# VealFang/PLI-SLAM

Hardware: AMD Instinct MI355X
Metric: stereo frames/sec (ORB+LSD extract+match), 752x480 EuRoC (higher is better)
Workload: dtype u8; 1 GPU; 1xMI355X: 752x480 stereo pairs, extract + stereo Hamming match (BASELINE configs[1] shape, batched); 752x480, 1200 ORB kp (8 levels x1.2) + LSD/LBD (<=100 lines); 256 stereo frames per GPU per step; frames_per_gpu=256, parallelism=frame-batch data parallel, 1 rank(s), gather of result tables to rank 0

## Files before the change

pli_slam_amd/csrc/common.hpp:

```cpp
#pragma once
#include <hip/hip_runtime.h>
#include <cstdint>
#include <cstdio>
#include <cstring>
#include <string>
#include <vector>
#include <map>
#include "../../include/pli_frontend.h"

namespace pli {

constexpr int MAX_LEVELS = 16;
constexpr int CELL_CAP = 512;
constexpr int GRID_COLS = 64;
constexpr int GRID_ROWS = 48;
constexpr int LSD_CHUNK = 4096;

struct LevelGeom {
  int w, h, pitch;
  int64_t offset;
  int minBX, minBY, maxBX, maxBY;
  int nCols, nRows, wCell, hCell;
  int cellBase;
  int nfeatures;
// ... 13 lines not shown
  LevelGeom lv[MAX_LEVELS];
  int cellsPerImage, kpSlotsPerImage, candPerImage;
  int64_t pyrBlock;
  int kpCap, klCap;
  int umax[16];
  int LW, LH, lpitch;
  int LWt;
  int g2Thresh;
  int nBins;
  int minRegSize;
  double prec, lsdScale;
  float alignLo, alignHi;
  double hotBand2;
  double rectApproxBand;
  int alignFilter, alignPad;
  int parityFlags, parityPad;
  double rho;
  int maxLines;
  int lsdNFeatures;
  double minLength;
  float bf, maxD;
  int sWs, bestLR;
  double lineSimTh, overlapTh, ratio12L, minDispRatio, minDisp, horizTh;
};

struct alignas(128) RxCtl {
  int state;
  int changed;
  int overflow;
  int rounds;
  int nSmall, nBig;
  int changedOdd;
  int pad0[25];
  int nHand;
  int pad1[31];
  int nextBig;
  int pad2[31];
  unsigned long long rectArena;
  int pad3[30];
  int races;
  int pad4[31];
};
constexpr int RX_ARENA_BITS = 40;

struct RxSeed {
  int rank, xy;
// ... 96 lines not shown
```

pli_slam_amd/csrc/lsd_rect.hpp:

```cpp
#pragma once
#include "kernels.hpp"
#include "device_prims.hpp"

namespace pli {

constexpr double RX_PI = 3.14159265358979323846;
constexpr double RX_DEG2RAD = RX_PI / 180;
constexpr double RX_3_2_PI = (3 * RX_PI) / 2;
constexpr double RX_2PI = 2 * RX_PI;

__device__ __forceinline__ double rx_angle_diff(double a, double b) {
  double diff = a - b;
  while (diff <= -RX_PI) diff += RX_2PI;
  while (diff > RX_PI) diff -= RX_2PI;
  return fabs(diff);
}

constexpr int RX_RECT_GROUP_MAX = 192;
constexpr int RX_RECT_CACHE = 4;

__device__ __forceinline__ void rx_wave_sync() {
  __builtin_amdgcn_fence(__ATOMIC_RELEASE, "wavefront");
  __builtin_amdgcn_wave_barrier();
  __builtin_amdgcn_fence(__ATOMIC_ACQUIRE, "wavefront");
}

template <int LANES>
__device__ __forceinline__ void rx_rect_region(bool on, const RxRect& it, const DevParams& P, const float4* __restrict__ rec,
                                               const double* __restrict__ mg, const int* __restrict__ arena,
                                               float4* __restrict__ rgSeg, double (*st)[64], double (*wc)[64], int (*ec)[64], int rmask,
                                               const int2* __restrict__ hot = nullptr ,
                                               const float2* __restrict__ cold = nullptr ) {
  const int lane = threadIdx.x & 63, gl = lane & (LANES - 1), g0 = lane & ~(LANES - 1);
  const int W = P.LW;
  const double prec = P.prec;
  const int cnt = on ? it.cnt : 0;
  const int* lst = arena + it.off;
  const double reg_angle = (double)fast_atan2_deg(it.sumdy, it.sumdx) * RX_DEG2RAD;
  int cmax = cnt;
#pragma unroll
  for (int o = 32; o >= LANES; o >>= 1) cmax = max(cmax, __shfl_xor(cmax, o, 64));
  double acc = 0.0;
  for (int c0 = 0; c0 < cmax; c0 += LANES) {
    const int kk = c0 + gl;
    double v0 = 0.0, v1 = 0.0, v2 = 0.0;
    if (kk < cnt) {
      const int e = lst[kk];
      const int ex = e & 0xFFFF, ey = e >> 16;
      const double w = mg ? mg[ey * W + ex] : sqrt((double)__float_as_int(rec[ey * W + ex].w) / 4.0);
      v0 = (double)ex * w;
      v1 = (double)ey * w;
      v2 = w;
      if (c0 < RX_RECT_CACHE * LANES) { wc[c0 / LANES][lane] = w; ec[c0 / LANES][lane] = e; }
    }
    rx_wave_sync();
    st[0][lane] = v0; st[1][lane] = v1; st[2][lane] = v2;
    rx_wave_sync();
    if (gl < 3 && c0 < cnt) {
      const int mm = (min(LANES, cnt - c0) + 7) & ~7;
      for (int tt = 0; tt < mm; tt += 8) {
        double a[8];
#pragma unroll
        for (int u = 0; u < 8; ++u) a[u] = st[gl][g0 + tt + u];
#pragma unroll
        for (int u = 0; u < 8; ++u) acc += a[u];
      }
    }
  }
  const double cq = acc / __shfl(acc, g0 + 2, 64);
  const double x = __shfl(cq, g0, 64), y = __shfl(cq, g0 + 1, 64);
  acc = 0.0;
  for (int c0 = 0; c0 < cmax; c0 += LANES) {
    const int kk = c0 + gl;
    double v0 = 0.0, v1 = 0.0, v2 = 0.0;
    if (kk < cnt) {
      const bool cached = c0 < RX_RECT_CACHE * LANES;
      const int e = cached ? ec[c0 / LANES][lane] : lst[kk];
      const int ex = e & 0xFFFF, ey = e >> 16;
      const double w = cached ? wc[c0 / LANES][lane] : (mg ? mg[ey * W + ex] : sqrt((double)__float_as_int(rec[ey * W + ex].w) / 4.0));
      const double dx = (double)ex - x, dy = (double)ey - y;
      v0 = dy * dy * w;
      v1 = dx * dx * w;
      v2 = dx * dy * w;
    }
    rx_wave_sync();
    st[0][lane] = v0; st[1][lane] = v1; st[2][lane] = v2;
    rx_wave_sync();
    if (gl < 3 && c0 < cnt) {
      const int mm = (min(LANES, cnt - c0) + 7) & ~7;
      for (int tt = 0; tt < mm; tt += 8) {
        double a[8];
#pragma unroll
        for (int u = 0; u < 8; ++u) a[u] = st[gl][g0 + tt + u];
        if (gl < 2) {
#pragma unroll
          for (int u = 0; u < 8; ++u) acc += a[u];
        } else {
#pragma unroll
          for (int u = 0; u < 8; ++u) acc -= a[u];
        }
      }
    }
  }
  const double Ixx = __shfl(acc, g0, 64), Iyy = __shfl(acc, g0 + 1, 64), Ixy = __shfl(acc, g0 + 2, 64);
  const double lambda = 0.5 * (Ixx + Iyy - sqrt((Ixx - Iyy) * (Ixx - Iyy) + 4.0 * Ixy * Ixy));
  const bool wide = fabs(Ixx) > fabs(Iyy);
  double theta = (double)fast_atan2_deg(wide ? (float)(lambda - Ixx) : (float)Ixy, wide ? (float)Ixy : (float)(lambda - Iyy));
  theta *= RX_DEG2RAD;
  double adiff = rx_angle_diff(theta, reg_angle);
  {
    const bool need = on && it.approx != 0 && hot != nullptr && fabs(adiff - prec) < P.rectApproxBand;
    if (__builtin_amdgcn_ballot_w64(need)) {
      int cm = need ? cnt : 0;
#pragma unroll
      for (int o = 32; o >= LANES; o >>= 1) cm = max(cm, __shfl_xor(cm, o, 64));
      float sx = 0.f, sy = 0.f;
      for (int c0 = 0; c0 < cm; c0 += LANES) {
        const int kk = c0 + gl;
        float cy = 0.f, cz = 0.f;
        if (need && kk < cnt) {
          const int e = lst[kk];
          const int p = (e >> 16) * W + (e & 0xFFFF);
          if (kk == 0) {
            double sn, cs;
            sincos((double)__int_as_float(hot[p].x) * RX_DEG2RAD, &sn, &cs);
// ... 23 lines not shown
  double l_min = 0, l_max = 0;
  for (int kk = gl; kk < cnt; kk += LANES) {
    const int e = kk < RX_RECT_CACHE * LANES ? ec[kk / LANES][lane] : lst[kk];
    const double l = ((double)(e & 0xFFFF) - x) * dxr + ((double)(e >> 16) - y) * dyr;
    l_max = fmax(l_max, l);
    l_min = fmin(l_min, l);
  }
#pragma unroll
  for (int o = LANES / 2; o > 0; o >>= 1) {
    l_max = fmax(l_max, __shfl_xor(l_max, o, 64));
    l_min = fmin(l_min, __shfl_xor(l_min, o, 64));
  }
  double e = ((gl & 1) ? y : x) + ((gl & 2) ? l_max : l_min) * ((gl & 1) ? dyr : dxr);
  e += 0.5;
  const double scale = P.lsdScale;
  if (scale != 1) e /= scale;
  if (on && gl < 4) reinterpret_cast<float*>(&rgSeg[it.rank & rmask])[gl] = (float)e;
}


__device__ __forceinline__ void rx_rect_wave(const DevParams& P, const RxCtl& c, const float4* __restrict__ rec, const double* __restrict__ mg,
                                             const int* __restrict__ arena, const RxRect* __restrict__ rects, int rectCap,
                                             float4* __restrict__ rgSeg, int first, int stride, double (*st)[64], double (*wc)[64],
                                             int (*ec)[64], int rmask = -1, const int2* __restrict__ hot = nullptr,
                                             const float2* __restrict__ cold = nullptr) {
  const int nrect = min((int)(c.rectArena >> RX_ARENA_BITS), rectCap);
  const int lane = threadIdx.x & 63, g = lane >> 4;
  for (int w0 = first * 4; w0 < nrect; w0 += stride * 4) {
    RxRect it = {0, 0, 0, 1.f, 0.f, 0};
    const bool have = w0 + g < nrect;
    if (have) it = rects[w0 + g];
    const bool small = have && it.cnt <= RX_RECT_GROUP_MAX;
    if (__builtin_amdgcn_ballot_w64(small)) rx_rect_region<16>(small, it, P, rec, mg, arena, rgSeg, st, wc, ec, rmask, hot, cold);
    unsigned long long big = __builtin_amdgcn_ballot_w64(have && !small) & 0x0001000100010001ull;
    while (big) {
      const int gl0 = __ffsll((long long)big) - 1;
      big &= big - 1ull;
      RxRect bt;
      bt.rank = __shfl(it.rank, gl0, 64); bt.off = __shfl(it.off, gl0, 64); bt.cnt = __shfl(it.cnt, gl0, 64);
      bt.sumdx = __shfl(it.sumdx, gl0, 64); bt.sumdy = __shfl(it.sumdy, gl0, 64); bt.approx = __shfl(it.approx, gl0, 64);
      rx_rect_region<64>(true, bt, P, rec, mg, arena, rgSeg, st, wc, ec, rmask, hot, cold);
    }
  }
}

}
```

pli_slam_amd/csrc/lsd_relax.hip:

```cpp
#include "kernels.hpp"
#include "device_prims.hpp"
#include "lsd_rect.hpp"
#include <climits>
#include <type_traits>

namespace pli {

constexpr float RX_NOTDEF = -1024.f;
constexpr int RX_INF = LSD_ID_INF;

__device__ __forceinline__ int2 rx_load_own(const int2* p) {
  unsigned long long v = __hip_atomic_load(reinterpret_cast<const unsigned long long*>(p), __ATOMIC_RELAXED,
                                           __HIP_MEMORY_SCOPE_AGENT);
  return make_int2((int)(v & 0xFFFFFFFFull), (int)(v >> 32));
}

__device__ __forceinline__ int rx_lds_read(const int* p) {
  typedef __attribute__((address_space(3))) const volatile int lds_cvint;
  return *(lds_cvint*)p;
}


__device__ __forceinline__ int rx_block_append(bool flag, int* counter, int* lds) {
  const int tid = threadIdx.x, lane = tid & 63, wv = tid >> 6, nw = blockDim.x >> 6;
// ... 674 lines not shown

__global__ __launch_bounds__(64) void k_rx_grow_wave(const DevParams* __restrict__ Pp, RxCtl* __restrict__ ctl,
                                                     const float4* __restrict__ recAll, int2* __restrict__ ownAll,
                                                     const RxSeed* __restrict__ bigAll, int bigCap,
                                                     const RxHand* __restrict__ handAll, int handCap,
                                                     int* __restrict__ rgSizeAll, int2* __restrict__ rgBoxAll,
                                                     int* __restrict__ arenaAll, int arenaCap,
                                                     RxRect* __restrict__ rectAll, int rectCap, int img0, int t) {
  rx_grow_groups<64, 1024>(Pp, ctl, recAll, ownAll, bigAll, bigCap, handAll, handCap, rgSizeAll, rgBoxAll, arenaAll, arenaCap,
                           rectAll, rectCap, img0, t);
}

#endif

__global__ __launch_bounds__(64) void k_rx_rect(const DevParams* __restrict__ Pp, RxCtl* __restrict__ ctl,
                                                const float4* __restrict__ recAll, const int* __restrict__ arenaAll,
                                                int arenaCap, const RxRect* __restrict__ rectAll, int rectCap,
                                                float4* __restrict__ rgSegAll, int img0, const double* __restrict__ mgAll, int rmask,
                                                const int2* __restrict__ hotAll ,
                                                const float2* __restrict__ coldAll ) {
  __shared__ double st[3][64];
  __shared__ double wc[RX_RECT_CACHE][64];
  __shared__ int ec[RX_RECT_CACHE][64];
  const DevParams& P = *Pp;
  const int img = blockIdx.y + img0;
  const RxCtl& c = ctl[img];
  if (c.state == 2 || c.overflow) return;
  const int64_t npix = (int64_t)P.LW * P.LH;
  rx_rect_wave(P, c, recAll + img * npix, mgAll ? mgAll + img * npix : nullptr ,
               arenaAll + (int64_t)img * arenaCap, rectAll + (int64_t)img * rectCap, rectCap, rgSegAll + img * npix, blockIdx.x, gridDim.x, st, wc, ec, rmask,
               hotAll ? hotAll + img * npix : nullptr, coldAll ? coldAll + img * npix : nullptr);
}

constexpr int RX_CCHUNK = 2048;

__device__ __forceinline__ bool rx_emits(const int* order, const int2* own, int size, int i, int n, int minReg) {
  if (i >= n) return false;
  return size >= minReg && own[order[i]].x == i;
}

__global__ __launch_bounds__(256) void k_rx_count(const RxCtl* __restrict__ ctl, const int* __restrict__ orderAll,
                                                  const int* __restrict__ nDefined, const int2* __restrict__ ownAll,
                                                  const int* __restrict__ rgSizeAll, int* __restrict__ chunkCntAll,
                                                  int nChunks, int64_t npix, int minReg, int img0) {
  __shared__ int wsum[4];
  const int img = blockIdx.y + img0;
  if (ctl[img].state != 2 || ctl[img].overflow) return;
  const int n = nDefined[img];
  const int tid = threadIdx.x;
  int cntv = 0;
  int sz[RX_CCHUNK / 256];
#pragma unroll
  for (int j = 0; j < RX_CCHUNK / 256; ++j) sz[j] = rgSizeAll[img * npix + min((int)blockIdx.x * RX_CCHUNK + j * 256 + tid, max(n - 1, 0))];
// ... 55 lines not shown
```

pli_slam_amd/csrc/lsd_tile.hip:

```cpp
#include "kernels.hpp"
#include "device_prims.hpp"
#include "lsd_rect.hpp"
#include <climits>
#include <type_traits>

namespace pli {

constexpr float TX_NOTDEF = -1024.f;
constexpr int TX_INF = LSD_ID_INF;
constexpr double TX_PI = 3.14159265358979323846;
constexpr double TX_DEG2RAD = TX_PI / 180;
constexpr double TX_3_2_PI = (3 * TX_PI) / 2;
constexpr double TX_2PI = 2 * TX_PI;
#if !defined(PLI_DEV) && (defined(TX_CLAIM_SCOPE) || defined(TX_GROUP) || defined(TX_OWN_LOAD) || defined(TX_DIAG_PAD) || defined(TX_DIAG_NOWAIT) || defined(TX_DIAG_HOT_NOFOLD))
#error "diagnostic builds of lsd_tile.hip need -DPLI_DEV"
#endif
#ifndef TX_CLAIM_SCOPE
#define TX_CLAIM_SCOPE __HIP_MEMORY_SCOPE_AGENT
#endif
#ifndef TX_GROUP
#define TX_GROUP 8
#endif
static_assert(TX_GROUP == 0 || TX_GROUP == 2 || TX_GROUP == 4 || TX_GROUP == 8, "a group member is an octet of lanes");
constexpr int TX_GQ = 768;
// ... 1965 lines not shown
    __builtin_amdgcn_fence(__ATOMIC_RELEASE, "agent");
    __hip_atomic_fetch_add(&bar[0], 1u, __ATOMIC_RELAXED, __HIP_MEMORY_SCOPE_AGENT);
    int ok = 1;
    unsigned spins = 0;
    while (__hip_atomic_load(&bar[0], __ATOMIC_RELAXED, __HIP_MEMORY_SCOPE_AGENT) < target) {
      __builtin_amdgcn_s_sleep(4);
      if ((++spins & 63u) == 0u &&
          (__hip_atomic_load(&bar[32], __ATOMIC_RELAXED, __HIP_MEMORY_SCOPE_AGENT) != 0u || spins > (1u << 21))) {
        __hip_atomic_store(&bar[32], 1u, __ATOMIC_RELAXED, __HIP_MEMORY_SCOPE_AGENT);
        ok = 0;
        break;
      }
    }
    __builtin_amdgcn_fence(__ATOMIC_ACQUIRE, "agent");
    s_ok = ok;
  }
  __syncthreads();
  asm volatile("s_dcache_inv" ::: "memory");
  return s_ok != 0;
}

__global__ __launch_bounds__(256) void k_tx_tail(TxTailArgs A) {
  __shared__ int qs[4][TX_GQ];
  __shared__ int gbs[4][TX_BMAXBLK + 4];
  __shared__ int parks[4][TX_PARK];
  __shared__ double sts[4][3][64];
  __shared__ double wcs[4][RX_RECT_CACHE][64];
  __shared__ int ecs[4][RX_RECT_CACHE][64];
  __shared__ int s_live, s_n;
  __shared__ int s_list[256];
  if (A.forceAbort) {
    if (threadIdx.x == 0) __hip_atomic_store(&A.bar[32], 1u, __ATOMIC_RELAXED, __HIP_MEMORY_SCOPE_AGENT);
    return;
  }
  const DevParams& P = *A.Pp;
  const int W = P.LW, H = P.LH;
  const int64_t npix = (int64_t)W * H;
  const int tid = threadIdx.x, wv = tid >> 6;
  const int G = gridDim.x;
  const int nbx = (W + 31) / 32, nbyA = (A.TH + 7) / 8, nbyB = (H + 31) / 32, ntile = A.ntx * A.nty, ncell = A.TW * A.TH;
  const int64_t nA = (int64_t)nbx * nbyA * A.nimg, nB = (int64_t)nbx * nbyB * A.nimg, nC = (int64_t)ntile * A.nimg;
  const int nwaves = G * 4, gw = blockIdx.x * 4 + wv;
  auto relaxing = [&](int il) -> bool {
    const RxCtl& c = A.ctl[A.img0 + il];
    return c.state != 2 && c.overflow == 0;
  };
// ... 79 lines not shown
        const int64_t va = base + (int64_t)s_list[i] * G;
        const int il = (int)(va / ntile);
        if (A.hot)
          tx_grow_tile<true, false, TX_GQ, 0, true>(A.Pp, A.ctl, A.rec, A.own, A.list, A.tileCnt, A.ts, A.ntx, A.nty, A.rgSize, A.rgBox, A.rgDirty,
                                                    A.tileAct, A.TW, A.TH, A.arena, A.arenaCap, A.rects, A.rectCap, A.img0 + il,
                                                    (int)(va - (int64_t)il * ntile), t, A.rank, A.rgLost, A.tileTouch, A.DL, qs[wv], gbs[wv],
                                                    parks[wv], nullptr, A.hot, A.cold);
        else
        tx_grow_tile<true>(A.Pp, A.ctl, A.rec, A.own, A.list, A.tileCnt, A.ts, A.ntx, A.nty, A.rgSize, A.rgBox, A.rgDirty, A.tileAct, A.TW,
                           A.TH, A.arena, A.arenaCap, A.rects, A.rectCap, A.img0 + il, (int)(va - (int64_t)il * ntile), t, A.rank, A.rgLost,
                           A.tileTouch, A.DL, qs[wv], gbs[wv], parks[wv]);
      }
      __syncthreads();
    }
    if (!tx_grid_barrier(A.bar, ++epoch * G)) return;
    for (int64_t v = (int64_t)blockIdx.x * 256 + tid; v < nC; v += (int64_t)G * 256) A.DL.cnt[(int64_t)A.img0 * ntile + v] = 0;
    {
      const int per = max(1, nwaves / A.nimg);
      for (int il = gw / per; il < A.nimg; il += max(1, nwaves / per)) {
        const int img = A.img0 + il;
        const RxCtl& c = A.ctl[img];
        if (c.state == 2 || c.overflow) continue;
        rx_rect_wave(P, c, A.rec + img * npix, A.mg ? A.mg + img * npix : nullptr, A.arena + (int64_t)img * A.arenaCap,
                     A.rects + (int64_t)img * A.rectCap, A.rectCap, A.rgSeg + img * npix, gw % per, per, sts[wv], wcs[wv], ecs[wv], A.DL.rmask,
                     A.hot ? A.hot + img * npix : nullptr, A.cold ? A.cold + img * npix : nullptr);
      }
    }
    if (!tx_grid_barrier(A.bar, ++epoch * G)) return;
  }
}

}
```

pli_slam_amd/csrc/pli_capi.hip:

```cpp
#include "kernels.hpp"
#include "scratch_plan.hpp"
#include <cmath>
#include <cfloat>
#include <algorithm>
#include <memory>
#include <limits>
#include <cstdlib>
#include <set>
#include <string>
#include <functional>
#include <mutex>
#include <atomic>
#include <dlfcn.h>

using namespace pli;

#ifdef PLI_DEV
#define DEVENV(name) getenv(name)
#else
static inline const char* pli_no_devenv() { return nullptr; }
#define DEVENV(name) (pli_no_devenv())
#endif

namespace {
// ... 6 lines not shown
    if (e__ != hipSuccess) {                                                                 \
      g_err = std::string(#expr) + ": " + hipGetErrorString(e__);                            \
      return PLI_ERR_HIP;                                                                    \
    }                                                                                        \
  } while (0)

inline int64_t alignUp(int64_t v, int64_t a) { return (v + a - 1) / a * a; }
inline int cvRoundf(float v) { return (int)std::nearbyintf(v); }
inline int cvRoundd(double v) { return (int)std::nearbyint(v); }
inline int cvFloorf(float v) { int i = (int)v; return i - (i > v); }

constexpr int RX_AUTO_IMAGES = 2560;
constexpr int TX_SMALL_TILE_WAVES = 12000;

struct ProfEntry { const char* name; hipEvent_t a, b; };

}

struct pli_ctx {
  mutable std::recursive_mutex mu;
  pli_frontend_config cfg;
  DevParams hp;
  DevParams* dP = nullptr;
  int device = 0;
  hipStream_t stream = nullptr;
  bool ownStream = true;
  hipStream_t aux = nullptr;
  hipEvent_t evFork = nullptr, evJoin = nullptr, evLbdPre = nullptr;
  hipStream_t aux2 = nullptr;
  hipEvent_t evRectFork = nullptr, evRectDone = nullptr;
  std::function<pli_status()> sideChain;
  bool lbdPreOnSide = false;
  bool syncDebug = getenv("PLI_SYNC_DEBUG") != nullptr;
  int NI = 0;
  pli_table_layout lay;
  std::vector<void*> allocs;
  uint8_t *pyr = nullptr, *blur = nullptr;
  int* resizeTab[MAX_LEVELS] = {nullptr};
  uint32_t* cellCand = nullptr; int* cellCount = nullptr;
  uint32_t* candAll = nullptr; unsigned short* nodeOf = nullptr; int* candCount = nullptr;
  uint32_t* kpSel = nullptr; int* kpSelCount = nullptr;
  BlurJob *jobOrb = nullptr, *jobLsd = nullptr, *jobLbd = nullptr;
  int orbTiles = 0, l0Tiles = 0;
  uint8_t *tmp8 = nullptr, *lsdScaled = nullptr;
  int64_t tmp8Stride = 0, lsdStride = 0;
  int tmpPitch = 0;
// ... 347 lines not shown
  L.kp_cap = kc; L.kl_cap = lc;
  L.off_counts = take(8 * 4);
  L.off_kp[0] = take((int64_t)kc * sizeof(pli_keypoint));
  L.off_kp[1] = take((int64_t)kc * sizeof(pli_keypoint));
  L.off_desc[0] = take((int64_t)kc * 32);
  L.off_desc[1] = take((int64_t)kc * 32);
  L.off_uright = take((int64_t)kc * 4);
  L.off_depth = take((int64_t)kc * 4);
  L.off_kl[0] = take((int64_t)lc * sizeof(pli_keyline));
  L.off_kl[1] = take((int64_t)lc * sizeof(pli_keyline));
  L.off_ldesc[0] = take((int64_t)lc * 32);
  L.off_ldesc[1] = take((int64_t)lc * 32);
  L.off_disp = take((int64_t)lc * 8);
  L.off_le = take((int64_t)lc * 24);
  L.record_bytes = alignUp(o, 256);
}

pli_status allocAll(pli_ctx* c) {
  const DevParams& P = c->hp;
  const int NI = c->NI;
  pli_status st;
#define A(ptr, n) if ((st = c->dalloc(&(ptr), (size_t)(n))) != PLI_OK) return st
  A(c->dP, 1);
  HIPCHK(hipMemcpy(c->dP, &c->hp, sizeof(DevParams), hipMemcpyHostToDevice));
  A(c->pyr, (size_t)P.pyrBlock * NI);
  for (int l = 1; l < P.nlevels; ++l) {
    const LevelGeom &S = P.lv[l - 1], &D = P.lv[l];
    std::vector<int> t = buildResizeTab(S.w, S.h, D.w, D.h, 1. / ((double)D.w / S.w), 1. / ((double)D.h / S.h));
    A(c->resizeTab[l], t.size());
    HIPCHK(hipMemcpy(c->resizeTab[l], t.data(), t.size() * 4, hipMemcpyHostToDevice));
  }
  A(c->cellCand, (size_t)NI * P.cellsPerImage * CELL_CAP);
  A(c->cellCount, (size_t)NI * P.cellsPerImage);
  A(c->candAll, (size_t)NI * P.candPerImage);
  A(c->nodeOf, (size_t)NI * P.candPerImage);
  A(c->candCount, (size_t)NI * P.nlevels);
  A(c->kpSel, (size_t)NI * P.kpSlotsPerImage);
  A(c->kpSelCount, (size_t)NI * P.nlevels);
  {
    BlurJob J;
    std::memset(&J, 0, sizeof(J));
    J.nplanes = P.nlevels;
    J.radius = ORB_BLUR_R;
    gaussKernelFixed8(2 * ORB_BLUR_R + 1, 2.0, J.k);
    {
      int ksum = 0, kmax = 0;
// ... 444 lines not shown
    if (items)
      LAUNCH(c, "k_lsd_rect", k_lsd_rect, dim3(16, nimg), dim3(64), 0, c->dP, (const LsdRectItem*)items, (const uint2*)c->regScratch,
             (const double*)c->mg, (const double*)c->rectW, (const int*)c->nSeg, c->seg, c->maxSeg, img0);
#endif
  } else {
    const bool trace = DEVENV("PLI_RX_TRACE") != nullptr;
    const bool fullPasses = DEVENV("PLI_RX_FULL") != nullptr;
    const bool perRound = DEVENV("PLI_RX_PROFROUNDS") != nullptr;
    int curT = 0;
    auto rxn = [&](const char* n) -> const char* {
      if (!perRound) return n;
      static std::set<std::string> pool;
      char b[64];
      std::snprintf(b, sizeof(b), "%s@%02d", n, curT);
      return pool.insert(b).first->c_str();
    };
    const int64_t npix64 = (int64_t)npix;
    int growBlocks = std::max(16, std::min(256, 2048 / nimg));
    if (const char* e = DEVENV("PLI_JR_BLOCKS")) growBlocks = std::max(1, atoi(e));
    int bigBlocks = std::max(64, std::min(1024, 16384 / nimg));
    if (const char* e = DEVENV("PLI_JR_BIGBLOCKS")) bigBlocks = std::max(1, atoi(e));
    int rectBlocks = std::max(64, std::min(2048, 32768 / nimg));
    if (const char* e = DEVENV("PLI_RECT_BLOCKS")) rectBlocks = std::max(1, atoi(e));
    int bigThresh = RX_HAND;
    if (const char* e = DEVENV("PLI_JR_BIG")) bigThresh = atoi(e);
    int maxRounds = 96;
    if (const char* e = DEVENV("PLI_RX_MAXROUNDS")) maxRounds = std::max(1, std::min(1 << 20, atoi(e)));
    const float precDeg = (float)(P.prec * 180.0 / 3.14159265358979323846);
    (void)growBlocks; (void)bigBlocks; (void)bigThresh; (void)precDeg;
    if (c->rgClean) HIPCHK(hipMemsetAsync(c->rgClean + (int64_t)img0 * npix, 0, npix64 * nimg, c->stream));
    const bool lostRule = c->lsdMode != 1 && DEVENV("PLI_TX_BOXRULE") == nullptr;
    {
      const int64_t cells = (int64_t)c->tilesW * c->tilesH;
      const int64_t ntile64 = (int64_t)c->txNtx * c->txNty;
      static_assert(sizeof(RxCtl) % 4 == 0, "RxCtl is cleared as words");
      ZeroRanges Z{};
      int zr = 0;
      constexpr int zmax = (int)(sizeof(Z.p) / sizeof(Z.p[0]));
      bool zfull = false;
      auto add = [&](void* p, int64_t words) {
        if (!p || words <= 0) return;
        if (zr == zmax) { zfull = true; return; }
        Z.p[zr] = (uint32_t*)p; Z.words[zr] = words; ++zr;
      };
      add(c->jrCtl + img0, (int64_t)(sizeof(RxCtl) / 4) * nimg);
      if (c->lsdMode == 1) add(c->rgDirty + (int64_t)img0 * npix, npix64 * nimg);
// ... 88 lines not shown
      bool useCells = fusedDM && DL.list && c->txCellList && (int64_t)c->tilesW * c->tilesH * nimg >= (1 << 20);
      if (const char* e = DEVENV("PLI_TX_CELLS")) useCells = atoi(e) != 0 && fusedDM && DL.list && c->txCellList;
      int tailT0 = useCells ? 12 : 8;
      if (const char* e = DEVENV("PLI_TX_TAIL_T0")) tailT0 = std::max(3, atoi(e));
      for (int t = 1; t <= maxRounds && !allDone; ++t) {
        curT = t;
        if (useTail && t == tailT0) {
          TxTailArgs ta{c->dP, c->jrCtl, c->rec, c->own, c->txList, c->txTileCnt, ts, c->txNtx, c->txNty, c->lastSize, c->rgBox, c->rgDirty,
                        c->tileAct, c->tileTouch, c->tilesW, c->tilesH, c->arena, c->arenaCap, c->rects, c->rectCap, c->rgSeg, c->mg,
                        c->rankOf, c->rgLost, DL, img0, nimg, t, maxRounds, c->tailBar};
          ta.hot = hotLater; ta.cold = coldPlane;
          int tb = std::min(c->tailBlocks, std::max(64, 8 * nimg));
          if (const char* e = DEVENV("PLI_TX_TAIL_BLOCKS")) tb = std::max(1, std::min(c->tailBlocks, atoi(e)));
          {
            std::lock_guard<std::mutex> lk(g_tailMu);
            hipEvent_t& ev = g_tailEv[c->device];
            c->tailLaunched = true;
            ta.forceAbort = DEVENV("PLI_TX_TAIL_FORCE_ABORT") ? 1 : 0;
            if (ev) HIPCHK(hipStreamWaitEvent(c->stream, ev, 0));
            else HIPCHK(hipEventCreateWithFlags(&ev, hipEventDisableTiming));
            LAUNCH(c, "k_tx_tail", k_tx_tail, dim3(tb), dim3(256), 0, ta);
            HIPCHK(hipEventRecord(ev, c->stream));
          }
          break;
        }
        if (t == 3 && DL.list && fullRound2)
          HIPCHK(hipMemsetAsync(c->txDirtyCnt + (int64_t)img0 * ntile, 0, sizeof(int) * (size_t)ntile * nimg, c->stream));
        const bool fused2 = t == 2 && !fullRound2 && lostRule && !DEVENV("PLI_TX_NOFUSE2");
        bool cellsDone = false;
        if (fused2) {
          TRL(c, "k_tx_round2", k_tx_round2, dim3((P.LW + 31) / 32, (P.LH + 31) / 32, nimg), dim3(256), 0, c->jrCtl, c->own, c->rankOf, c->order,
              c->rgBox, c->rgDirty, c->tileAct, P.LW, P.LH, c->tilesW, c->tilesH, t, img0, (const int*)c->rgLost, DL, c->tileTouch,
              (pack1 && !hotPlane) ? (const float4*)c->rec : (const float4*)nullptr, rectAside ? 1 : 0, (const int2*)hotPlane);
          if (rectAside) {
            HIPCHK(hipStreamWaitEvent(c->stream, c->evRectDone, 0));
            TRL(c, "k_tx_reset_rect", k_tx_reset_rect, dim3((nimg + 255) / 256), dim3(256), 0, c->jrCtl, nimg, img0);
          }
          if (c->sideChain && sideForkRound == -2) {
            auto f = std::move(c->sideChain);
            c->sideChain = nullptr;
            pli_status ss = f();
            if (ss != PLI_OK) return ss;
          }
        } else if (t >= 3 && fusedDM && useCells && t < TX_CELL_ROUNDS) {
          const int ncell = c->tilesW * c->tilesH;
          const dim3 lg((unsigned)((ncell + 2047) / 2048), nimg), wg((unsigned)(4 * std::max(8, std::min(256, std::max(ncell / 1024, 4096 / nimg)))), nimg);
// ... 106 lines not shown
            HIPCHK(hipStreamCreateWithFlags(&c->aux2, hipStreamNonBlocking));
            rectS = c->aux2;
          }
          hipStream_t mainS = c->stream;
          HIPCHK(hipEventRecord(c->evRectFork, mainS));
          HIPCHK(hipStreamWaitEvent(rectS, c->evRectFork, 0));
          c->stream = rectS;
          hipError_t le = hipSuccess;
          {
            auto launchRect = [&]() -> pli_status {
              TRL(c, "k_rx_rect", k_rx_rect, dim3(rectBlocks, nimg), dim3(64), 0, c->dP, c->jrCtl, c->rec, c->arena, c->arenaCap, c->rects,
                  c->rectCap, c->rgSeg, img0, c->mg, DL.rmask, (const int2*)hotPlane, (const float2*)coldPlane);
              return PLI_OK;
            };
            const pli_status rs = launchRect();
            c->stream = mainS;
            if (rs != PLI_OK) return rs;
          }
          (void)le;
          HIPCHK(hipEventRecord(c->evRectDone, rectS));
        } else
        TRL(c, "k_rx_rect", k_rx_rect, dim3(rectBlocks, nimg), dim3(64), 0, c->dP, c->jrCtl, c->rec, c->arena, c->arenaCap, c->rects,
            c->rectCap, c->rgSeg, img0, c->mg, DL.rmask, (const int2*)hotPlane, (const float2*)coldPlane);
        if (trace) {
          HIPCHK(hipMemcpyAsync(c->jrHost.data(), c->jrCtl + img0, sizeof(RxCtl) * nimg, hipMemcpyDeviceToHost, c->stream));
          HIPCHK(hipStreamSynchronize(c->stream));
          const RxCtl& h = c->jrHost[0];
          std::fprintf(stderr, "[tx] t=%d state=%d changed=%d overflow=%d rect=%d arena=%lld\n", t, h.state, h.changed, h.overflow,
                       (int)(h.rectArena >> RX_ARENA_BITS), (long long)(h.rectArena & ((1ull << RX_ARENA_BITS) - 1ull)));
        }
        pli_status ls = look(t);
        if (ls != PLI_OK) return ls;
      }
    } else {
#ifndef PLI_DEV
      g_err = "lsd_mode 1 (the lane relaxation) is a development schedule: libpli_frontend_dev.so";
      return PLI_ERR_INVALID;
#else
    TRL(c, "k_rx_guess", k_rx_guess, raster, dim3(256), 0, c->rec, c->rankOf, c->own, P.LW, P.LH, precDeg, img0);
    for (int t = 1; t <= maxRounds && !allDone; ++t) {
      curT = t;
      TRL(c, "k_rx_diff", k_rx_diff, dim3((P.LW + 31) / 32, (c->tilesH + 7) / 8, nimg), dim3(256), 0, c->jrCtl, c->own, c->tileMin, c->tileAct,
             P.LW, P.LH, c->tilesW, c->tilesH, t, img0, (const int*)nullptr);
      if (t >= 3 && !fullPasses) {
        TRL(c, "k_rx_mark", k_rx_mark, dim3((P.LW + 31) / 32, (c->tilesH + 7) / 8, nimg), dim3(256), 0, c->jrCtl, c->own, c->rankOf, c->rgBox,
            c->rgDirty, c->tileMin, c->tileAct, P.LW, P.LH, c->tilesW, c->tilesH, t, img0, 1, (const int*)nullptr, TxDirtyLists{});
// ... 1627 lines not shown
      const int64_t np = (int64_t)P.LW * P.LH;
      if (!need(np * 4)) return dst ? PLI_ERR_CAPACITY : PLI_OK;
      HIPCHK(hipMemcpy(dst, c->lastSize + image * np, np * 4, hipMemcpyDeviceToHost));
      return PLI_OK;
    }
    case PLI_DBG_STEREO_SAD: {
      const int frame = image >> 1;
      const int64_t n = (int64_t)P.kpCap * 4;
      if (!need(2 * n)) return dst ? PLI_ERR_CAPACITY : PLI_OK;
      HIPCHK(hipMemcpy(dst, c->sad + (int64_t)frame * P.kpCap, n, hipMemcpyDeviceToHost));
      HIPCHK(hipMemcpy((char*)dst + n, c->bestIdx + (int64_t)frame * P.kpCap, n, hipMemcpyDeviceToHost));
      return PLI_OK;
    }
    default:
      g_err = "unknown debug item";
      return PLI_ERR_INVALID;
  }
}

}

#ifdef PLI_DEV
extern "C" int32_t pli_dev_orb_window_reach(void) { return ORB_REACH; }
#endif
```

Baseline: 6440 stereo frames/s.

## Sort LSD rectangle regions by chunk count per wave and prefetch region loads

Each wave now loads a batch of up to 64 rectangle records, buckets them by chunk count with ballots, and writes them to shared memory in sorted order. Small regions are then processed four per wave with similar sizes grouped together, and large regions are handled one per wave, which is meant to cut lane idling caused by mismatched region sizes. The region moment computation now issues its list and weight loads ahead of use: up to four cached chunks are loaded up front, and later chunks are software-pipelined two chunks ahead. Dev-only histogram counters are added behind PLI_DEV. The cost is extra shared memory (64 RxRect entries, reusing the grower queue inside k_tx_tail), ballot and sort overhead per batch, and more register pressure.

After: 6484 stereo frames/s (median of 6 runs). About the same (+0.7%).

```diff
diff --git a/pli_slam_amd/csrc/common.hpp b/pli_slam_amd/csrc/common.hpp
--- a/pli_slam_amd/csrc/common.hpp
+++ b/pli_slam_amd/csrc/common.hpp
@@ -59,6 +59,9 @@
   float bf, maxD;
   int sWs, bestLR;
   double lineSimTh, overlapTh, ratio12L, minDispRatio, minDisp, horizTh;
+#ifdef PLI_DEV
+  unsigned long long* rectHist;
+#endif
 };
 
 struct alignas(128) RxCtl {
diff --git a/pli_slam_amd/csrc/lsd_rect.hpp b/pli_slam_amd/csrc/lsd_rect.hpp
--- a/pli_slam_amd/csrc/lsd_rect.hpp
+++ b/pli_slam_amd/csrc/lsd_rect.hpp
@@ -31,6 +31,7 @@
                                                float4* __restrict__ rgSeg, double (*st)[64], double (*wc)[64], int (*ec)[64], int rmask,
                                                const int2* __restrict__ hot = nullptr ,
                                                const float2* __restrict__ cold = nullptr ) {
+  constexpr int C = RX_RECT_CACHE;
   const int lane = threadIdx.x & 63, gl = lane & (LANES - 1), g0 = lane & ~(LANES - 1);
   const int W = P.LW;
   const double prec = P.prec;
@@ -40,19 +41,22 @@
   int cmax = cnt;
 #pragma unroll
   for (int o = 32; o >= LANES; o >>= 1) cmax = max(cmax, __shfl_xor(cmax, o, 64));
+  cmax = __builtin_amdgcn_readfirstlane(cmax);
+  auto ldE = [&](int c0) __attribute__((always_inline)) -> int {
+    const int kk = c0 + gl;
+    const int e = lst[kk < cnt ? kk : 0];
+    return cnt > 0 ? e : 0;
+  };
+  auto ldW = [&](int e, bool norm) __attribute__((always_inline)) -> double {
+    const int p = (e >> 16) * W + (e & 0xFFFF);
+    return norm ? mg[p] : sqrt((double)__float_as_int(rec[p].w) / 4.0);
+  };
+  int e1 = 0, e2 = 0;
+  double w1 = 0.0;
+  int e1s = 0, e2s = 0;
+  double w1s = 0.0;
   double acc = 0.0;
-  for (int c0 = 0; c0 < cmax; c0 += LANES) {
-    const int kk = c0 + gl;
-    double v0 = 0.0, v1 = 0.0, v2 = 0.0;
-    if (kk < cnt) {
-      const int e = lst[kk];
-      const int ex = e & 0xFFFF, ey = e >> 16;
-      const double w = mg ? mg[ey * W + ex] : sqrt((double)__float_as_int(rec[ey * W + ex].w) / 4.0);
-      v0 = (double)ex * w;
-      v1 = (double)ey * w;
-      v2 = w;
-      if (c0 < RX_RECT_CACHE * LANES) { wc[c0 / LANES][lane] = w; ec[c0 / LANES][lane] = e; }
-    }
+  auto chunk_sum = [&](int c0, double v0, double v1, double v2, bool sub) __attribute__((always_inline)) {
     rx_wave_sync();
     st[0][lane] = v0; st[1][lane] = v1; st[2][lane] = v2;
     rx_wave_sync();
@@ -62,45 +66,104 @@
         double a[8];
 #pragma unroll
         for (int u = 0; u < 8; ++u) a[u] = st[gl][g0 + tt + u];
-#pragma unroll
-        for (int u = 0; u < 8; ++u) acc += a[u];
-      }
-    }
+        if (!sub || gl < 2) {
+#pragma unroll
+          for (int u = 0; u < 8; ++u) acc += a[u];
+        } else {
+#pragma unroll
+          for (int u = 0; u < 8; ++u) acc -= a[u];
+        }
+      }
+    }
+  };
+  auto rest = [&](auto prod, bool sub) __attribute__((always_inline)) {
+    for (int c0 = C * LANES; c0 < cmax; c0 += LANES) {
+      const int e = e1;
+      const double w = w1;
+      e1 = e2;
+      e2 = ldE(c0 + 2 * LANES);
+      w1 = ldW(e1, mg != nullptr);
+      double v0, v1, v2;
+      prod(e, w, c0 + gl < cnt, v0, v1, v2);
+      chunk_sum(c0, v0, v1, v2, sub);
+    }
+  };
+  {
+    auto prod = [&](int e, double w, bool ok, double& v0, double& v1, double& v2) __attribute__((always_inline)) {
+      const int ex = e & 0xFFFF, ey = e >> 16;
+      v0 = ok ? (double)ex * w : 0.0;
+      v1 = ok ? (double)ey * w : 0.0;
+      v2 = ok ? w : 0.0;
+    };
+    static_assert(C == 4, "the cached chunks are written out one by one");
+    int eA = 0, eB = 0, eD = 0, eF = 0;
+    double wA = 0.0, wB = 0.0, wD = 0.0, wF = 0.0;
+    auto loads = [&](int n, bool norm) __attribute__((always_inline)) {
+      eA = ldE(0 * LANES);
+      if (n > 1) eB = ldE(1 * LANES);
+      if (n > 2) eD = ldE(2 * LANES);
+      if (n > 3) eF = ldE(3 * LANES);
+      if (n > 4) { e1 = ldE(4 * LANES); e2 = ldE(5 * LANES); }
+      wA = ldW(eA, norm);
+      if (n > 1) wB = ldW(eB, norm);
+      if (n > 2) wD = ldW(eD, norm);
+      if (n > 3) wF = ldW(eF, norm);
+      if (n > 4) w1 = ldW(e1, norm);
+    };
+    if (mg) {
+      if (cmax > 4 * LANES) loads(5, true);
+      else if (cmax > 3 * LANES) loads(4, true);
+      else if (cmax > 2 * LANES) loads(3, true);
+      else if (cmax > 1 * LANES) loads(2, true);
+      else loads(1, true);
+    } else {
+      if (cmax > 4 * LANES) loads(5, false);
+      else if (cmax > 3 * LANES) loads(4, false);
+      else if (cmax > 2 * LANES) loads(3, false);
+      else if (cmax > 1 * LANES) loads(2, false);
+      else loads(1, false);
+    }
+    auto cached = [&](int c, int e, double w) __attribute__((always_inline)) {
+      if (c * LANES < cmax) {
+        const bool ok = c * LANES + gl < cnt;
+        if (ok) { wc[c][lane] = w; ec[c][lane] = e; }
+        double v0, v1, v2;
+        prod(e, w, ok, v0, v1, v2);
+        chunk_sum(c * LANES, v0, v1, v2, false);
+      }
+    };
+    cached(0, eA, wA);
+    cached(1, eB, wB);
+    cached(2, eD, wD);
+    cached(3, eF, wF);
+    e1s = e1; e2s = e2; w1s = w1;
+    rest(prod, false);
   }
   const double cq = acc / __shfl(acc, g0 + 2, 64);
   const double x = __shfl(cq, g0, 64), y = __shfl(cq, g0 + 1, 64);
   acc = 0.0;
-  for (int c0 = 0; c0 < cmax; c0 += LANES) {
-    const int kk = c0 + gl;
-    double v0 = 0.0, v1 = 0.0, v2 = 0.0;
-    if (kk < cnt) {
-      const bool cached = c0 < RX_RECT_CACHE * LANES;
-      const int e = cached ? ec[c0 / LANES][lane] : lst[kk];
+  {
+    auto prod = [&](int e, double w, bool ok, double& v0, double& v1, double& v2) __attribute__((always_inline)) {
       const int ex = e & 0xFFFF, ey = e >> 16;
-      const double w = cached ? wc[c0 / LANES][lane] : (mg ? mg[ey * W + ex] : sqrt((double)__float_as_int(rec[ey * W + ex].w) / 4.0));
       const double dx = (double)ex - x, dy = (double)ey - y;
-      v0 = dy * dy * w;
-      v1 = dx * dx * w;
-      v2 = dx * dy * w;
-    }
-    rx_wave_sync();
-    st[0][lane] = v0; st[1][lane] = v1; st[2][lane] = v2;
-    rx_wave_sync();
-    if (gl < 3 && c0 < cnt) {
-      const int mm = (min(LANES, cnt - c0) + 7) & ~7;
-      for (int tt = 0; tt < mm; tt += 8) {
-        double a[8];
-#pragma unroll
-        for (int u = 0; u < 8; ++u) a[u] = st[gl][g0 + tt + u];
-        if (gl < 2) {
-#pragma unroll
-          for (int u = 0; u < 8; ++u) acc += a[u];
-        } else {
-#pragma unroll
-          for (int u = 0; u < 8; ++u) acc -= a[u];
-        }
-      }
-    }
+      v0 = ok ? dy * dy * w : 0.0;
+      v1 = ok ? dx * dx * w : 0.0;
+      v2 = ok ? dx * dy * w : 0.0;
+    };
+    e1 = e1s; e2 = e2s; w1 = w1s;
+#pragma unroll
+    for (int c = 0; c < C; ++c) {
+      if (c * LANES < cmax) {
+        const bool ok = c * LANES + gl < cnt;
+        int e = 0;
+        double w = 0.0;
+        if (ok) { e = ec[c][lane]; w = wc[c][lane]; }
+        double v0, v1, v2;
+        prod(e, w, ok, v0, v1, v2);
+        chunk_sum(c * LANES, v0, v1, v2, true);
+      }
+    }
+    rest(prod, true);
   }
   const double Ixx = __shfl(acc, g0, 64), Iyy = __shfl(acc, g0 + 1, 64), Ixy = __shfl(acc, g0 + 2, 64);
   const double lambda = 0.5 * (Ixx + Iyy - sqrt((Ixx - Iyy) * (Ixx - Iyy) + 4.0 * Ixy * Ixy));
@@ -170,26 +233,66 @@
 __device__ __forceinline__ void rx_rect_wave(const DevParams& P, const RxCtl& c, const float4* __restrict__ rec, const double* __restrict__ mg,
                                              const int* __restrict__ arena, const RxRect* __restrict__ rects, int rectCap,
                                              float4* __restrict__ rgSeg, int first, int stride, double (*st)[64], double (*wc)[64],
-                                             int (*ec)[64], int rmask = -1, const int2* __restrict__ hot = nullptr,
+                                             int (*ec)[64], RxRect* so ,
+                                             int rmask = -1, const int2* __restrict__ hot = nullptr,
                                              const float2* __restrict__ cold = nullptr) {
   const int nrect = min((int)(c.rectArena >> RX_ARENA_BITS), rectCap);
   const int lane = threadIdx.x & 63, g = lane >> 4;
-  for (int w0 = first * 4; w0 < nrect; w0 += stride * 4) {
-    RxRect it = {0, 0, 0, 1.f, 0.f, 0};
-    const bool have = w0 + g < nrect;
-    if (have) it = rects[w0 + g];
-    const bool small = have && it.cnt <= RX_RECT_GROUP_MAX;
-    if (__builtin_amdgcn_ballot_w64(small)) rx_rect_region<16>(small, it, P, rec, mg, arena, rgSeg, st, wc, ec, rmask, hot, cold);
-    unsigned long long big = __builtin_amdgcn_ballot_w64(have && !small) & 0x0001000100010001ull;
-    while (big) {
-      const int gl0 = __ffsll((long long)big) - 1;
-      big &= big - 1ull;
-      RxRect bt;
-      bt.rank = __shfl(it.rank, gl0, 64); bt.off = __shfl(it.off, gl0, 64); bt.cnt = __shfl(it.cnt, gl0, 64);
-      bt.sumdx = __shfl(it.sumdx, gl0, 64); bt.sumdy = __shfl(it.sumdy, gl0, 64); bt.approx = __shfl(it.approx, gl0, 64);
-      rx_rect_region<64>(true, bt, P, rec, mg, arena, rgSeg, st, wc, ec, rmask, hot, cold);
-    }
-  }
-}
-
-}
+  const int B = min(64, max(4, ((nrect + stride - 1) / stride + 3) & ~3));
+  constexpr int KBIG = RX_RECT_GROUP_MAX / 16 + 1, KNONE = KBIG + 1;
+#ifdef PLI_DEV
+  if (P.rectHist && lane == 0 && nrect > 0) {
+    atomicAdd(&P.rectHist[10], 1ull);
+    if (first * B >= nrect) atomicAdd(&P.rectHist[9], 1ull);
+    if (first == 0 && nrect % 4 != 0 && nrect % 64 != 0) atomicAdd(&P.rectHist[13], 1ull);
+    if (first == 0 && nrect < 4) atomicAdd(&P.rectHist[14], 1ull);
+  }
+#endif
+  for (int b0 = first * B; b0 < nrect; b0 += stride * B) {
+    const int n = min(B, nrect - b0);
+    const bool have = lane < n;
+    const RxRect& it = rects[b0 + (have ? lane : 0)];
+    const int rank = it.rank, off = it.off, cnt = it.cnt, approx = it.approx;
+    const float sumdx = it.sumdx, sumdy = it.sumdy;
+    const int ch = (cnt + 15) >> 4;
+    const int key = !have ? KNONE : cnt > RX_RECT_GROUP_MAX ? KBIG : ch;
+    int pos = 0, base = 0, nsmall = 0;
+    for (int i = 0; i <= KNONE; ++i) {
+      const int k = i < KBIG ? KBIG - 1 - i : i;
+      if (i == KBIG) nsmall = base;
+      const unsigned long long m = __builtin_amdgcn_ballot_w64(key == k);
+      if (key == k) pos = base + __builtin_amdgcn_mbcnt_hi((unsigned)(m >> 32), __builtin_amdgcn_mbcnt_lo((unsigned)m, 0u));
+      base += __popcll(m);
+    }
+    rx_wave_sync();
+    so[pos].rank = rank; so[pos].off = off; so[pos].cnt = cnt; so[pos].sumdx = sumdx; so[pos].sumdy = sumdy; so[pos].approx = approx;
+    rx_wave_sync();
+#ifdef PLI_DEV
+    if (P.rectHist) {
+      const int cls = cnt <= 16 ? 0 : cnt <= 32 ? 1 : cnt <= 48 ? 2 : cnt <= 64 ? 3 : cnt <= RX_RECT_GROUP_MAX ? 4 : 5;
+      unsigned long long add[9];
+      for (int k = 0; k < 6; ++k) add[k] = (unsigned long long)__popcll(__builtin_amdgcn_ballot_w64(have && cls == k));
+      const int own = key < KBIG ? ch : 0;
+      int lq = max(own, __shfl_xor(own, 1, 64));
+      lq = max(lq, __shfl_xor(lq, 2, 64));
+      const int sch = lane < nsmall ? (so[lane].cnt + 15) >> 4 : 0;
+      add[6] = (unsigned long long)wave_sum_i32((lane & 3) == 0 ? lq : 0);
+      add[7] = (unsigned long long)wave_sum_i32(own);
+      add[8] = (unsigned long long)wave_sum_i32((lane & 3) == 0 ? sch : 0);
+      const unsigned long long n256 = (unsigned long long)__popcll(__builtin_amdgcn_ballot_w64(have && cnt > 256));
+      const unsigned long long n1000 = (unsigned long long)__popcll(__builtin_amdgcn_ballot_w64(have && cnt > 1000));
+      if (lane == 0) {
+        for (int k = 0; k < 9; ++k)
+          if (add[k]) atomicAdd(&P.rectHist[k], add[k]);
+        if (n256) atomicAdd(&P.rectHist[11], n256);
+        if (n1000) atomicAdd(&P.rectHist[12], n1000);
+      }
+    }
+#endif
+    const int nbig = __popcll(__builtin_amdgcn_ballot_w64(key == KBIG));
+    for (int q0 = 0; q0 < nsmall; q0 += 4) rx_rect_region<16>(q0 + g < nsmall, so[q0 + g], P, rec, mg, arena, rgSeg, st, wc, ec, rmask, hot, cold);
+    for (int i = nsmall; i < nsmall + nbig; ++i) rx_rect_region<64>(true, so[i], P, rec, mg, arena, rgSeg, st, wc, ec, rmask, hot, cold);
+  }
+}
+
+}
diff --git a/pli_slam_amd/csrc/lsd_relax.hip b/pli_slam_amd/csrc/lsd_relax.hip
--- a/pli_slam_amd/csrc/lsd_relax.hip
+++ b/pli_slam_amd/csrc/lsd_relax.hip
@@ -720,13 +720,14 @@
   __shared__ double st[3][64];
   __shared__ double wc[RX_RECT_CACHE][64];
   __shared__ int ec[RX_RECT_CACHE][64];
+  __shared__ RxRect ordered[64];
   const DevParams& P = *Pp;
   const int img = blockIdx.y + img0;
   const RxCtl& c = ctl[img];
   if (c.state == 2 || c.overflow) return;
   const int64_t npix = (int64_t)P.LW * P.LH;
   rx_rect_wave(P, c, recAll + img * npix, mgAll ? mgAll + img * npix : nullptr ,
-               arenaAll + (int64_t)img * arenaCap, rectAll + (int64_t)img * rectCap, rectCap, rgSegAll + img * npix, blockIdx.x, gridDim.x, st, wc, ec, rmask,
+               arenaAll + (int64_t)img * arenaCap, rectAll + (int64_t)img * rectCap, rectCap, rgSegAll + img * npix, blockIdx.x, gridDim.x, st, wc, ec, ordered, rmask,
                hotAll ? hotAll + img * npix : nullptr, coldAll ? coldAll + img * npix : nullptr);
 }
 
diff --git a/pli_slam_amd/csrc/lsd_tile.hip b/pli_slam_amd/csrc/lsd_tile.hip
--- a/pli_slam_amd/csrc/lsd_tile.hip
+++ b/pli_slam_amd/csrc/lsd_tile.hip
@@ -2011,6 +2011,7 @@
 
 __global__ __launch_bounds__(256) void k_tx_tail(TxTailArgs A) {
   __shared__ int qs[4][TX_GQ];
+  static_assert(sizeof(int) * TX_GQ >= sizeof(RxRect) * 64, "the rect phase orders a block of 64 entries in the growers' queue");
   __shared__ int gbs[4][TX_BMAXBLK + 4];
   __shared__ int parks[4][TX_PARK];
   __shared__ double sts[4][3][64];
@@ -2136,7 +2137,8 @@
         const RxCtl& c = A.ctl[img];
         if (c.state == 2 || c.overflow) continue;
         rx_rect_wave(P, c, A.rec + img * npix, A.mg ? A.mg + img * npix : nullptr, A.arena + (int64_t)img * A.arenaCap,
-                     A.rects + (int64_t)img * A.rectCap, A.rectCap, A.rgSeg + img * npix, gw % per, per, sts[wv], wcs[wv], ecs[wv], A.DL.rmask,
+                     A.rects + (int64_t)img * A.rectCap, A.rectCap, A.rgSeg + img * npix, gw % per, per, sts[wv], wcs[wv], ecs[wv],
+                     reinterpret_cast<RxRect*>(qs[wv]) , A.DL.rmask,
                      A.hot ? A.hot + img * npix : nullptr, A.cold ? A.cold + img * npix : nullptr);
       }
     }
diff --git a/pli_slam_amd/csrc/pli_capi.hip b/pli_slam_amd/csrc/pli_capi.hip
--- a/pli_slam_amd/csrc/pli_capi.hip
+++ b/pli_slam_amd/csrc/pli_capi.hip
@@ -52,6 +52,9 @@
   pli_frontend_config cfg;
   DevParams hp;
   DevParams* dP = nullptr;
+#ifdef PLI_DEV
+  unsigned long long* rectHist = nullptr;
+#endif
   int device = 0;
   hipStream_t stream = nullptr;
   bool ownStream = true;
@@ -445,6 +448,11 @@
   pli_status st;
 #define A(ptr, n) if ((st = c->dalloc(&(ptr), (size_t)(n))) != PLI_OK) return st
   A(c->dP, 1);
+#ifdef PLI_DEV
+  A(c->rectHist, 16);
+  HIPCHK(hipMemset(c->rectHist, 0, 16 * sizeof(unsigned long long)));
+  c->hp.rectHist = c->rectHist;
+#endif
   HIPCHK(hipMemcpy(c->dP, &c->hp, sizeof(DevParams), hipMemcpyHostToDevice));
   A(c->pyr, (size_t)P.pyrBlock * NI);
   for (int l = 1; l < P.nlevels; ++l) {
@@ -935,6 +943,20 @@
     if (const char* e = DEVENV("PLI_JR_BIGBLOCKS")) bigBlocks = std::max(1, atoi(e));
     int rectBlocks = std::max(64, std::min(2048, 32768 / nimg));
     if (const char* e = DEVENV("PLI_RECT_BLOCKS")) rectBlocks = std::max(1, atoi(e));
+#ifdef PLI_DEV
+    const bool rectHistLines = DEVENV("PLI_RECT_HIST") != nullptr;
+    auto rectHistLine = [&](const char* what, int t) -> pli_status {
+      if (!rectHistLines) return PLI_OK;
+      unsigned long long h[16];
+      HIPCHK(hipDeviceSynchronize());
+      HIPCHK(hipMemcpy(h, c->rectHist, sizeof(h), hipMemcpyDeviceToHost));
+      HIPCHK(hipMemset(c->rectHist, 0, sizeof(h)));
+      std::fprintf(stderr, "[rect] %s t=%d images=%d regions by chunks 1:%llu 2:%llu 3:%llu 4:%llu 5-12:%llu wave:%llu  quad trips list-order %llu "
+                   "matched %llu (groups' own %llu)  wave shares empty %llu of %llu\n", what, t, nimg, h[0], h[1], h[2], h[3], h[4], h[5], h[6],
+                   h[8], h[7], h[9], h[10]);
+      return PLI_OK;
+    };
+#endif
     int bigThresh = RX_HAND;
     if (const char* e = DEVENV("PLI_JR_BIG")) bigThresh = atoi(e);
     int maxRounds = 96;
@@ -1069,6 +1091,9 @@
             LAUNCH(c, "k_tx_tail", k_tx_tail, dim3(tb), dim3(256), 0, ta);
             HIPCHK(hipEventRecord(ev, c->stream));
           }
+#ifdef PLI_DEV
+          { pli_status hs = rectHistLine("k_tx_tail", t); if (hs != PLI_OK) return hs; }
+#endif
           break;
         }
         if (t == 3 && DL.list && fullRound2)
@@ -1221,6 +1246,9 @@
         } else
         TRL(c, "k_rx_rect", k_rx_rect, dim3(rectBlocks, nimg), dim3(64), 0, c->dP, c->jrCtl, c->rec, c->arena, c->arenaCap, c->rects,
             c->rectCap, c->rgSeg, img0, c->mg, DL.rmask, (const int2*)hotPlane, (const float2*)coldPlane);
+#ifdef PLI_DEV
+        { pli_status hs = rectHistLine("k_rx_rect", t); if (hs != PLI_OK) return hs; }
+#endif
         if (trace) {
           HIPCHK(hipMemcpyAsync(c->jrHost.data(), c->jrCtl + img0, sizeof(RxCtl) * nimg, hipMemcpyDeviceToHost, c->stream));
           HIPCHK(hipStreamSynchronize(c->stream));
@@ -2894,4 +2922,17 @@
 
 #ifdef PLI_DEV
 extern "C" int32_t pli_dev_orb_window_reach(void) { return ORB_REACH; }
+
+extern "C" int32_t pli_dev_rect_hist(pli_ctx* c, uint64_t out[16], int32_t reset) {
+  CtxGuard guard__(c);
+  if (!c || !out) { g_err = "bad argument"; return PLI_ERR_INVALID; }
+  HIPCHK(hipSetDevice(c->device));
+  HIPCHK(hipStreamSynchronize(c->stream));
+  if (c->aux) HIPCHK(hipStreamSynchronize(c->aux));
+  if (c->aux2) HIPCHK(hipStreamSynchronize(c->aux2));
+  static_assert(sizeof(unsigned long long) == sizeof(uint64_t), "counter width");
+  HIPCHK(hipMemcpy(out, c->rectHist, 16 * sizeof(uint64_t), hipMemcpyDeviceToHost));
+  if (reset) HIPCHK(hipMemset(c->rectHist, 0, 16 * sizeof(uint64_t)));
+  return PLI_OK;
+}
 #endif
```
